# brucefan1983/GPUMD

Measured on AMD Instinct MI355X. Metric: atom-steps/sec, NEP PbTe NVE (nep4 2 Te Pb, examples/nep_train/nep.txt), higher is better.
Workload: dtype f32

## Files before the change

### gpumd_amd/csrc/capi_impl.h

```cpp
#pragma once
#include "../../include/nepmi.h"
#include "engine_impl.h"

#include <exception>
#include <string>

struct nepmi_api;
#if defined(NEPMI_CAPI_DISPATCH)
extern "C" const nepmi_api nepmi_self_api;
#define NEPMI_SELF_API (&nepmi_self_api)
#else
#define NEPMI_SELF_API nullptr
#endif

struct nepmi_model {
  const nepmi_api* api;
  nepmi::NepModel m;
};

struct nepmi_engine {
  const nepmi_api* api;
  nepmi::EngineT<NepmiBackend>* e;
};

// ... 903 lines not shown
int nepmi_engine_set_option(nepmi_engine* e, const char* name, double value)
{
  if (!e || !name)
    return fail(NEPMI_ERR_ARG, "null engine or option name");
  const std::string n(name);
  const int iv = (int)value;
  auto& eng = *e->e;
  if (n == "generic")
    return guarded([&] { eng.set_force_generic(iv != 0); });
  if (n == "tiles")
    eng.set_tile_mode(iv < 0 ? -1 : iv > 2 ? 2 : iv);
  else if (n == "win_lanes")
    eng.set_win_lanes(iv);
  else if (n == "win_max_atoms")
    eng.set_win_max_atoms(iv);
  else if (n == "scatter_guard")
    eng.set_scatter_guard_delayed(value, eng.take_guard_delay());
  else if (n == "scatter_guard_hard")
    eng.set_scatter_guard(-1.0, value);
  else if (n == "scatter_guard_delay")
    eng.set_guard_delay(iv);
  else if (n == "radial_mask")
    eng.set_radial_mask(iv != 0);
  else if (n == "radial_sync")
    eng.set_radial_sync(iv != 0);
  else if (n == "angular_fused")
    eng.set_angular_fused(iv != 0);
  else if (n == "angular_pair_trip")
    eng.set_angular_pair_trip(iv != 0);
  else if (n == "angular_flat_tables")
    eng.set_angular_flat_tables(iv != 0);
  else if (n == "lean_list_walks")
    eng.set_lean_list_walks(iv != 0);
  else if (n == "fold_seam")
    eng.set_fold_seam(iv != 0);
  else if (n == "brick_force") {
    if (iv != 0 && !eng.has_brick_force())
      return fail(NEPMI_ERR_ARG, "option 'brick_force': the per-brick force kernel is not part of this build (make BRICK=1)");
    eng.set_brick_force(iv != 0);
  }
  else if (n == "win_static")
    eng.set_win2(iv != 0);
  else if (n == "keep_lists_on_box_change")
    eng.set_keep_lists(iv != 0);
  else if (n == "stepwise_loops")
    eng.set_stepwise_loops(iv != 0);
  else if (n == "mfma")
    eng.set_use_mfma(iv);
  else if (n == "angular_recompute")
    eng.set_angular_recompute(iv);
  else
    return fail(NEPMI_ERR_ARG, "unknown engine option '" + n + "'");
  return NEPMI_OK;
}

}
```

### gpumd_amd/csrc/engine_impl.h

```cpp
#pragma once
#include "nep_bodies.h"
#include "nep_md.h"
#include "nep_corr.h"
#include "nep_rdf.h"
#include "nep_adf.h"
#include "nep_model.h"
#include "nep_window.h"
#include "nep_highl.h"
#include "tersoff_bodies.h"

#include <cmath>
#include <cstdio>
#include <cstring>
#include <string>
#include <random>
#include <vector>

#ifndef NEPMI_TERSOFF_SEAM
#define NEPMI_TERSOFF_SEAM 1
#endif
#ifndef NEPMI_WIN2_DEFAULT
#define NEPMI_WIN2_DEFAULT 1
#endif

// ... 1216 lines not shown
    b_.posq = dalloc<PosQ>(N);
    b_.x0s = dalloc<double>(3 * N);
    b_.nn_skin = dalloc<int>(N);
    b_.nl_skin = dalloc<int>((size_t)b_.MN_skin * N);
    b_.code_skin = dalloc<unsigned short>((size_t)b_.MN_skin * N);
    b_.nn_ang = dalloc<int>(N);
    b_.nl_ang = dalloc<int>((size_t)b_.MN_ang * N);
    b_.code_ang = dalloc<unsigned short>((size_t)b_.MN_ang * N);
    b_.rev_ang = dalloc<unsigned short>((size_t)b_.MN_ang * N);
    b_.nn_rad = dalloc<int>(N);
    b_.nn_angstep = dalloc<int>(N);
    b_.nn_angtrue = dalloc<int>(N);
    if (m.kind == 0) {
      b_.rstash = dalloc<F4>((size_t)(b_.MN_ang + b_.MN_skin) * N);
      b_.acomp = dalloc<F4>((size_t)b_.MN_arows * N);
      b_.amap = dalloc<unsigned short>((size_t)b_.MN_ang * N);
      b_.f12 = dalloc<F4>((size_t)b_.MN_arows * N);
      b_.q = dalloc<float>((size_t)m.dim * N);
      b_.fp = dalloc<float>((size_t)m.dim * N);
      b_.sbuf = dalloc<float>((size_t)(m.n_max_angular + 1) * kNumHarm * N);
      b_.shi = m.L_max > 4 ? dalloc<float>((size_t)(m.n_max_angular + 1) * kHighSums * N) : nullptr;
      b_.KRP = ((m.basis_size_radial + 1) + 3) / 4 * 4;
      b_.atab = dalloc<float>((size_t)N * m.num_types * b_.KRP);
      const AnnMfmaShape as = ann_mfma_shape(m.num_types, m.dim, m.num_neurons, b_.KRP);
      b_.ann_img = as.ok ? dalloc<float>(as.img_floats * m.num_types) : nullptr;
      be_.ann_prepare(md_, b_);
      b_.pe_i = dalloc<float>(N);
      b_.MN_rad = m.MN_radial;
      b_.ccode = dalloc<unsigned short>((size_t)b_.MN_rad * N);
      b_.nn_t0 = dalloc<int>(N);
      b_.prec = dalloc<WinRec>(N);
      b_.aidx = dalloc<unsigned short>((size_t)b_.MN_acomp * N);
      b_.amask = dalloc<unsigned>(4 * (size_t)N);
      b_.MN_wchunks = (b_.MN_ang + 3) / 4 + 2 * ((b_.MN_skin + 3) / 4) + 4;
      b_.wcode = dalloc<unsigned short>((size_t)b_.MN_wchunks * 4 * N);
      b_.wseg = dalloc<int>(N);
      b_.FPR = (m.n_max_radial + 1 + 3) / 4 * 4;
      b_.fpr = (m.num_types > 4 || !served_by_type_pure_shape(m)) ? dalloc<float>((size_t)N * b_.FPR) : nullptr;
      b_.MN_cw = (b_.MN_rad + 3) / 4 + 1;
      b_.cword = dalloc<unsigned short>((size_t)2 * b_.MN_cw * 4 * N);
      b_.aslot = B::kHasScatter ? dalloc<unsigned short>((size_t)b_.MN_arows * N) : nullptr;
      b_.compact_all = b_.aslot ? 1 : 0;
      b_.MAW = (4 * ((b_.MN_ang + 3) / 4) + 31) / 32 + 1;
      b_.MBW = (8 * ((b_.MN_skin + 3) / 4) + 31) / 32 + 1;
      b_.rmaskA = B::kHasScatter ? dalloc<unsigned>((size_t)b_.MAW * N) : nullptr;
      b_.rmaskB = B::kHasScatter ? dalloc<unsigned>((size_t)b_.MBW * N) : nullptr;
      b_.tmaskA = B::kHasScatter ? dalloc<unsigned>((size_t)b_.MAW * N) : nullptr;
      b_.MA2 = 2 * ((b_.MN_ang + 3) / 4) + 2;
      const bool two = B::kHasScatter && m.num_types == 2;
      b_.acode2 = two ? dalloc<unsigned short>((size_t)b_.MA2 * N * 4) : nullptr;
      b_.aorig2 = two ? dalloc<unsigned>((size_t)b_.MA2 * N) : nullptr;
      b_.aseg2 = two ? dalloc<int>(N) : nullptr;
      b_.use_rmask = 0;
      b_.use_csync = 0;
    } else {
      tb_.rec = dalloc<D4>((size_t)b_.MN_ang * N);
      tb_.bb = dalloc<double>((size_t)b_.MN_ang * N);
      tb_.bp = dalloc<double>((size_t)b_.MN_ang * N);
      tb_.f12 = dalloc<D4>((size_t)b_.MN_ang * N);
      tb_.pe_d = dalloc<double>(N);
      tb_.mask = dalloc<unsigned long long>(N);
      for (int k = 0; k < 3; ++k) {
        const TersoffSet& s = m.ters[k];
        tp_.p[k] = TersoffSetD{s.a, s.b, s.lambda, s.mu, s.beta, s.n, s.c, s.d, s.h, s.r1, s.r2, s.c2, s.d2,
                               s.one_plus_c2overd2, s.pi_factor, s.minus_half_over_n};
      }
      tp_.rc_sq = (float)(m.rc_radial_max * m.rc_radial_max);
// ... 260 lines not shown
      build_in_windows = flags[kFlagMaxCell] <= 127 && flags[kFlagMaxWindow] <= win_max_atoms() && !flags[kFlagOutlier];
      for (int d = 0; d < 3; ++d)
        if (box_.pbc[d] && nb[d] < 8)
          build_in_windows = false;
      if (build_in_windows) {
        WinLayout lay = win_;
        lay.wmax = (flags[kFlagMaxWindow] + 63) / 64 * 64;
        lay.compact = 0;
        be_.launch_win(kSlotMisc, num_bricks_, BuildListsWinBody{WinStage{box_, b_, lay}});
      }
    }
    if (!build_in_windows)
      be_.template launch<128>(kSlotMisc, N_, BuildListsBody{box_, b_});
    rev_valid_ = false;
    if (model_.kind == 1 || b_.level)
      ensure_reverse_slots();
    be_.end_region(kRegionRebuild);
    be_.d2h(flags, b_.flags, sizeof(flags));
    check_overflow(flags);
    num_boundary_bricks_ = flags[kFlagNumBoundary];
    max_ang_rebuild_ = flags[kFlagMaxAng];
    tile_ok_ = use_tiles_ && model_.kind == 0 && flags[kFlagMaxCell] <= 127 && flags[kFlagMaxWindow] <= win_max_atoms() &&
               !flags[kFlagOutlier];
    for (int d = 0; d < 3; ++d)
      if (box_.pbc[d] && nb[d] < 8)
        tile_ok_ = false;
    if (std::getenv("NEPMI_DEBUG_REBUILD"))
      std::fprintf(stderr, "nepmi rebuild: cells %d %d %d max_cell %d max_window %d (cap %d) max_brick %d outlier %d tiles %d -> tile_ok %d\n", nb[0], nb[1], nb[2],
                   flags[kFlagMaxCell], flags[kFlagMaxWindow], win_max_atoms(), flags[kFlagMaxBrick], flags[kFlagOutlier], (int)use_tiles_, (int)tile_ok_);
    win_.wmax = (flags[kFlagMaxWindow] + 63) / 64 * 64;
    win2_ok_ = tile_ok_ && use_win2_ && b_.wtab != nullptr && win_.wmax < 65535;
    if (win2_ok_) {
      b_.wsent = win_.wmax;
      be_.template launch<128>(kSlotMisc, N_, PackCodesBody{b_, shape_ts() == 2 ? 2 : 1});
      be_.d2h(flags, b_.flags, sizeof(flags));
      check_overflow(flags);
    }
    if (win2_ok_ && b_.aslot) {
      const size_t need = (size_t)num_bricks_ * (size_t)win_.wmax * kHaloRowWords;
      if (need > halo_cap_) {
        dfree(halo_);
        halo_ = nullptr;
        halo_ = dalloc<int>(need + need / 8);
        halo_cap_ = need + need / 8;
      }
      if (!fmap_)
        fmap_ = dalloc<unsigned>((size_t)fold_rows_ * cap_);
      fold_ok_ = num_bricks_ < ((int64_t)1 << 19) && win_.wmax < (1 << 13);
      if (fold_ok_) {
        int most = be_.build_fold_map(N_, box_, b_, win_.wmax, fold_rows_, fmap_);
        if (most > fold_rows_) {
          fold_rows_ = most;
          dfree(fmap_);
          fmap_ = nullptr;
          fmap_ = dalloc<unsigned>((size_t)fold_rows_ * cap_);
          most = be_.build_fold_map(N_, box_, b_, win_.wmax, fold_rows_, fmap_);
        }
      }
    }
    if (reverse_ghosts_ && b_.level) {
      be_.memset(b_.atab, 0, sizeof(float) * (size_t)cap_ * model_.num_types * b_.KRP);
      be_.memset(b_.f12, 0, sizeof(F4) * (size_t)b_.MN_arows * cap_);
      if (b_.fpr)
        be_.memset(b_.fpr, 0, sizeof(float) * (size_t)cap_ * b_.FPR);
    }
    have_list_ = true;
    ++num_rebuild;
// ... 299 lines not shown
    if (!m.temperature_model || m.kind != 0 || temperature == temperature_)
      return;
    temperature_ = temperature;
    const float qT = (float)temperature * m.q_scaler_temp;
    b0_eff_.resize(m.b0.size());
    for (size_t k = 0; k < m.b0.size(); ++k)
      b0_eff_[k] = m.b0[k] - m.w0_temp[k] * qT;
    be_.h2d(const_cast<float*>(md_.b0), b0_eff_.data(), sizeof(float) * b0_eff_.size());
    be_.ann_prepare(md_, b_);
    fused_img_stale_ = fused_img_flat_stale_ = true;
  }
  double temperature() const { return temperature_; }
  bool temperature_model() const { return model_.temperature_model; }
  int recompute_s() const
  {
    return recompute_mode_ < 0 ? (model_.MN_angular <= 16 ? 1 : 0) : (recompute_mode_ ? 1 : 0);
  }
  void adopt_from(const EngineT& o)
  {
    use_tiles_ = o.use_tiles_;
    tile_mode_ = o.tile_mode_;
    recompute_mode_ = o.recompute_mode_;
    win_lanes_ = o.win_lanes_;
    win_max_atoms_ = o.win_max_atoms_;
    use_win2_ = o.use_win2_;
    external_skin_ = o.external_skin_;
    force_form_ = o.force_form_;
    use_rmask_ = o.use_rmask_;
    use_csync_ = o.use_csync_;
    ang_fused_ = o.ang_fused_;
    ang_pair_trip_ = o.ang_pair_trip_;
    ang_flat_tables_ = o.ang_flat_tables_;
    lean_walks_ = o.lean_walks_;
    fold_seam_ = o.fold_seam_;
    brick_force_ = o.brick_force_;
    loop_ctx_ = o.loop_ctx_;
    scatter_disabled_ = o.scatter_disabled_;
    b_.scatter_limit = o.b_.scatter_limit;
    b_.fold_guard = o.b_.fold_guard;
    b_.scatter_hard = o.b_.scatter_hard;
    b_.fold_hard = o.b_.fold_hard;
    hard_factor_ = o.hard_factor_;
    hard_asked_ = o.hard_asked_;
    guard_delay_ = o.guard_delay_;
    guard_delayed_ = o.guard_delayed_;
    if (reverse_ghosts_ != o.reverse_ghosts_)
      set_reverse_ghosts(o.reverse_ghosts_);
    unwrapped_ = o.unwrapped_;
    nhc_fresh_ = o.nhc_fresh_;
    bdp_rng_ = o.bdp_rng_;
    bdp_iset_ = o.bdp_iset_;
    bdp_gset_ = o.bdp_gset_;
    lan_seed_ = o.lan_seed_;
    num_compute = o.num_compute;
    num_rebuild = o.num_rebuild;
    num_discarded = o.num_discarded;
    num_range_handovers = o.num_range_handovers;
    be_.adopt_options(o.be_);
    if (ann_mode_ != o.ann_mode_)
      set_use_mfma(o.ann_mode_);
    if (force_generic_ != o.force_generic_)
      set_force_generic(o.force_generic_);
    if (o.temperature_ != temperature_)
      set_temperature(o.temperature_);
    have_list_ = false;
  }
// ... 45 lines not shown
      be_.template launch<64>(kSlotMisc, N_, RadialDescBody<S>{box_, md_, b_, 1});
      records_valid_ = true;
      return;
    }
    const int lanes = win_lanes();
    const bool win2 = win2_ok_ && lanes == 1;
    last_rows_form_ = false;
    last_fpj_form_ = false;
    if (phase != kPhaseRadialOnly) {
      WinLayout layq = win_;
      layq.compact = 1;
      const WinStage wsq{box_, b_, layq};
      b_.use_rmask = (NEPMI_RMASK && use_rmask_ && S::TS > 0 && win2 && b_.rmaskB && loop_ctx_ && max_ang_rebuild_ <= 96 &&
                      (S::TS == 1 || b_.acode2) && scatter_wanted<S>(wsq))
                       ? 1
                       : 0;
      last_mask_form_ = b_.use_rmask != 0;
      b_.use_csync = (NEPMI_CSYNC && use_csync_ && !b_.use_rmask && win2 && b_.cword && loop_ctx_ && b_.MN_cw < 256 &&
                      scatter_wanted<S>(wsq))
                       ? 1
                       : 0;
      last_sync_form_ = b_.use_csync != 0;
    } else {
      b_.use_rmask = 0;
      b_.use_csync = 0;
    }
    WinLayout lay2 = win_;
    lay2.compact = 1;
    const WinStage ws2{box_, b_, lay2};
    if (!(win2 && b_.use_csync && S::fixed))
      ensure_reverse_slots();
    B& rbe = radial_side_ ? *radial_side_ : be_;
    auto radial = [&](int64_t nb, int first) {
      if (win2 && b_.use_csync && lean_radial<S>())
        rbe.launch_win2(kSlotRadial, nb, RadialWin2Body<S, 1, 1>{ws2, md_, first, frozen});
      else if (win2 && b_.use_csync)
        rbe.launch_win2(kSlotRadial, nb, RadialWin2Body<S, 1>{ws2, md_, first, frozen});
      else if (win2 && lean_radial<S>())
        rbe.launch_win2(kSlotRadial, nb, RadialWin2Body<S, 0, 1>{ws2, md_, first, frozen});
      else if (win2)
        rbe.launch_win2(kSlotRadial, nb, RadialWin2Body<S>{ws2, md_, first, frozen});
      else if (lanes == 4)
        rbe.launch_win_split(kSlotRadial, nb, RadialWinSplitBody<S, 4>{ws, md_, first, frozen});
      else if (lanes == 2)
        rbe.launch_win_split(kSlotRadial, nb, RadialWinSplitBody<S, 2>{ws, md_, first, frozen});
      else
        rbe.launch_win(kSlotRadial, nb, RadialWinBody<S>{ws, md_, first, frozen});
    };
    if (phase == kPhaseRadialOnly) {
      b_.use_rmask = 0;
      b_.use_csync = 0;
      if (tile_ok_)
        radial(num_bricks_, -1);
      ccode_valid_ = true;
      return;
    }
    if (phase == kPhaseInterior) {
      radial(num_bricks_ - num_boundary_bricks_, 0);
      return;
    }
    if (phase == kPhaseBoundaryRadial) {
      radial(num_boundary_bricks_, (int)(num_bricks_ - num_boundary_bricks_));
      return;
    }
    records_valid_ = !tile_ok_;
    be_.begin_region(kRegionForce);
// ... 146 lines not shown
      fold_deferred_ = true;
    } else {
      be_.template launch_force_scatter<S>(kSlotForce, num_bricks_, -1, N_, ws2, md_, halo_, fmap_, fold_rows_, step_outputs_,
                                           list_mode(), 0, 2, frozen);
    }
    if (!step_outputs_)
      outputs_stale_ = true;
    last_scatter_form_ = true;
    return true;
  }
  template <class S>
  void assembly_rest_shape(const int* frozen)
  {
    WinLayout lay2 = win_;
    lay2.compact = 1;
    const WinStage ws2{box_, b_, lay2};
    be_.template launch_force_scatter<S>(kSlotForce, num_bricks_ - num_boundary_bricks_, 0, N_, ws2, md_, halo_, fmap_, fold_rows_,
                                         pending_outputs_, list_mode(), 2, 2, frozen);
  }

public:
  void set_force_form(int mode) { force_form_ = mode < 0 ? -1 : (mode > 1 ? 1 : mode); }
  void set_assembly_part(int part) { assembly_part_ = part; }
  bool assembly_pending() const { return assembly_pending_; }
  void force_assembly_rest(const int* frozen)
  {
    if (!assembly_pending_)
      return;
    assembly_pending_ = false;
    be_.frozen = frozen;
    NEPMI_SHAPE_DISPATCH(assembly_rest_shape, 1, (frozen))
    be_.frozen = nullptr;
  }
  void set_radial_mask(bool on) { use_rmask_ = on; }
  void set_radial_sync(bool on) { use_csync_ = on; }
  void set_scatter_guard(double limit, double hard_factor = 4.0)
  {
    if (limit < 0.0)
      limit = b_.scatter_limit;
    if (hard_factor >= 0.0)
      hard_asked_ = hard_factor;
    if (!(limit > 0.0) || limit > 64.0)
      limit = 64.0;
    hard_factor = hard_asked_;
    if (!(hard_factor >= 1.0) || hard_factor * limit > 256.0)
      hard_factor = 256.0 / limit < 4.0 ? 256.0 / limit : 4.0;
    b_.scatter_limit = (float)limit;
    b_.fold_guard = (int)(2.0 * limit * 4194304.0);
    hard_factor_ = hard_factor;
    if (b_.scatter_hard > 0.0f)
      set_flagged_steps_stand(true);
  }
  double scatter_guard() const { return b_.scatter_limit; }
  void set_scatter_guard_delayed(double limit, int n)
  {
    if (n <= 0) {
      set_scatter_guard(limit, -1.0);
      return;
    }
    guard_delayed_ = limit;
    guard_delay_ = n;
  }
  void set_guard_delay(int n) { guard_delay_next_ = n > 0 ? n : 0; }
  int take_guard_delay()
  {
    const int n = guard_delay_next_;
    guard_delay_next_ = 0;
    return n;
  }
  void set_flagged_steps_stand(bool on)
  {
    b_.scatter_hard = on ? (float)(hard_factor_ * b_.scatter_limit) : 0.0f;
    b_.fold_hard = on ? (int)((hard_factor_ > 2.0 ? hard_factor_ : 2.0) * b_.scatter_limit * 4194304.0) : 0;
  }
  bool scatter_enabled() const { return !scatter_disabled_; }
  void clear_range_hard()
  {
    int ov = 0;
    be_.d2h(&ov, b_.flags + kFlagOverflow, sizeof(int));
    if (ov & kOverflowRangeHard) {
      ov &= ~kOverflowRangeHard;
      be_.h2d(b_.flags + kFlagOverflow, &ov, sizeof(int));
    }
  }
  void disable_scatter()
  {
    if (!scatter_disabled_)
      ++num_range_handovers;
    scatter_disabled_ = true;
    be_.memset(b_.flags + kFlagRange, 0, sizeof(int));
  }
  bool last_scatter_form() const { return last_scatter_form_; }
  void set_angular_fused(bool on) { ang_fused_ = on; }
  void set_angular_pair_trip(bool on) { ang_pair_trip_ = on; }
  bool ang_pair_trip_active() const { return ang_pair_trip_ && (model_.n_max_angular + 2) / 2 <= 4; }
  void set_angular_flat_tables(bool on) { ang_flat_tables_ = on; }
  void set_lean_list_walks(bool on) { lean_walks_ = on; }
  template <class S>
  bool lean_radial() const
  {
    return lean_walks_ && S::TS > 0;
  }
  bool lean_scatter() const { return lean_walks_ && shape_ts() > 0; }
  void set_fold_seam(bool on) { fold_seam_ = on; }
  void set_brick_force(bool on) { brick_force_ = on; }
  static constexpr bool has_brick_force() { return B::kHasBrickForce; }
  void set_loop_context(bool on) { loop_ctx_ = on; }
  void set_step_outputs(bool on) { step_outputs_ = on; }
  bool loop_context() const { return loop_ctx_; }
  void exact_virials()
  {
    if (!virial_local_ || model_.kind != 0 || last_small_)
      return;
    be_.frozen = nullptr;
    NEPMI_SHAPE_DISPATCH(exact_virials_shape, 1, ())
  }
  bool virial_local() const { return virial_local_; }

private:
  template <class S>
  void compact_lists_shape()
  {
    const bool padded_rows = b_.use_csync != 0;
    force_kernels_shape<S>(kPhaseRadialOnly, nullptr);
    if (padded_rows)
      angular_kernels<S>();
  }
  template <class S>
  void exact_virials_shape()
  {
// ... 72 lines not shown
          char eb[128];
          std::snprintf(eb, sizeof eb, "<-zero_padded_model(%d,%d,%d,%d,%d)", model_.file_n_max_radial, model_.file_basis_size_radial,
                        model_.file_n_max_angular, model_.file_basis_size_angular, model_.file_num_L);
          s += eb;
        }
      } else {
        s += std::string("shape=") + shapes[shape_ >= 0 && shape_ <= 5 ? shape_ : 0];
      }
    }
    if (last_small_)
      return s + " path=small_box(all image pairs)";
    const int lanes = win_lanes();
    const bool win2 = win2_ok_ && lanes == 1;
    s += tile_ok_ ? (win2 ? " window=lds_static" : " window=lds_scanned") : " window=none(gather kernels)";
    s += " lanes_per_atom=" + std::to_string(tile_ok_ ? lanes : 1);
    if (last_brick_)
      s += " force=one_kernel_per_brick(descriptor+ann+partial_forces+lds_scatter_of_own_halves,lane_pairs)";
    else if (last_ang_fused_ && last_ang_window_)
      s += " angular=descriptor+ann+partial_forces_in_one_kernel(lane_pairs,sums_in_registers,type_sorted,window_of_4_types)";
    else if (last_ang_fused_)
      s += std::string(" angular=descriptor+ann+partial_forces_in_one_kernel(lane_pairs,sums_in_registers") +
           (ang_pair_trip_active() ? ",two_record_trips" : "") + (last_ang_flat_ ? ",flat_tables)" : ")");
    else if (fuse_ann_active())
      s += " ann=fused_with_angular_descriptor(packed_fp32,no_mfma)";
    else if (ann_mode_ != 0 && b_.ann_img && (model_.num_types <= 4 || b_.skip_atab))
      s += model_.num_types > 4 ? " ann=mfma_f32_32x32x2(one_type_per_workgroup)" : " ann=mfma_f32_32x32x2";
    else
      s += " ann=per_atom";
    if (!last_ang_fused_) {
      s += (shape_ != 0 && model_.n_max_angular + 1 >= 7) ? " angular_force=lane_pairs" : " angular_force=one_lane";
      s += recompute_s() ? " angular_sums=recomputed" : " angular_sums=stored";
    }
    s += (tile_ok_ && win2 && shape_ts() > 0 && lean_walks_) ? " list_walks=lean" : " list_walks=classic";
    s += (last_scatter_form_ && last_mask_form_)   ? " radial_list=inside_bits_over_the_verlet_words"
         : (last_scatter_form_ && last_sync_form_) ? " radial_list=wave_synchronous_words"
                                                   : " radial_list=compacted";
    s += last_scatter_form_ ? (last_fold_seam_ ? " force_assembly=lds_scatter_of_own_halves(fixed_point)+fold_in_integrator_pass"
                                               : " force_assembly=lds_scatter_of_own_halves(fixed_point)+fold") :
         last_rows_form_ ? " force_assembly=table_rows_in_lds"
                         : (last_fpj_form_ ? " force_assembly=neighbour_half_from_fp_rows" : " force_assembly=table_rows_gathered");
    if (num_seam_vetoes_ > 0)
      s += " seam_vetoes=" + std::to_string(num_seam_vetoes_);
    if (tile_ok_)
      s += " bricks=" + std::to_string(num_bricks_) + " window_slots=" + std::to_string(win_.wmax);
    return s;
  }
  void force_kernels(int phase, const int* frozen = nullptr)
  {
    be_.frozen = frozen;
    force_kernels_dispatch(phase, frozen);
    be_.frozen = nullptr;
    step_outputs_ = true;
    assembly_part_ = 0;
  }
  void force_kernels_on(B& side, int phase, const int* frozen)
  {
    if (phase != kPhaseBoundaryRadial || !tile_ok_)
      throw EngineError{-4, "force_kernels_on: the boundary bricks' radial pass of the window kernels only"};
    radial_side_ = &side;
    side.frozen = frozen;
    force_kernels_dispatch(phase, frozen);
    side.frozen = nullptr;
    radial_side_ = nullptr;
  }

private:
// ... 4 lines not shown
      if (N_ < 200000)
        be_.template launch_lds_parts<kTersoffBlock, kTersoffLanes>(kSlotRadial, N_, TersoffPartialBody{box_, tp_, b_, tb_, kTersoffLanes});
      else
        be_.template launch_lds<kTersoffBlock>(kSlotRadial, N_, TersoffPartialBody{box_, tp_, b_, tb_});
      if (tersoff_defer_)
        tersoff_deferred_ = true;
      else
        be_.template launch<64>(kSlotForce, N_, TersoffAssembleBody{b_, tb_});
      be_.end_region(kRegionForce);
      return;
    }
    NEPMI_SHAPE_DISPATCH(force_kernels_shape, 1, (phase, frozen))
  }

  NepModel model_;
  B be_;
  int64_t cap_;
  int64_t N_;
  ModelD md_{};
  Bufs b_;
  BoxD box_;
  WinLayout win_{0, 0};
  bool win2_ok_ = false, use_win2_ = NEPMI_WIN2_DEFAULT != 0;
  bool use_rows_ = true;
  bool last_rows_form_ = false, last_fpj_form_ = false, last_scatter_form_ = false;
  int force_form_ = -1;
  bool loop_ctx_ = false;
  bool virial_local_ = false;
  double hard_factor_ = 4.0;
  bool ang_fused_ = true;
  bool ang_pair_trip_ = !(std::getenv("NEPMI_ANGULAR_PAIR_TRIP") && std::atoi(std::getenv("NEPMI_ANGULAR_PAIR_TRIP")) == 0);
  bool ang_flat_tables_ = !(std::getenv("NEPMI_ANGULAR_FLAT_TABLES") && std::atoi(std::getenv("NEPMI_ANGULAR_FLAT_TABLES")) == 0);
  bool lean_walks_ = !(std::getenv("NEPMI_LEAN_LIST_WALKS") && std::atoi(std::getenv("NEPMI_LEAN_LIST_WALKS")) == 0);
  float* fused_img_flat_ = nullptr;
  size_t fused_img_flat_floats_ = 0;
  bool fused_img_flat_stale_ = true;
  bool last_ang_flat_ = false;
  bool brick_force_ = false;
  bool last_brick_ = false;
  bool brick_pending_ = false;
  float* fused_img_ = nullptr;
  size_t fused_img_floats_ = 0;
  bool fused_img_stale_ = true;
  bool last_ang_fused_ = false;
  bool use_rmask_ = false;
  bool last_mask_form_ = false;
  bool last_ang_window_ = false;
  bool last_sync_form_ = false;
  int guard_delay_ = 0;
  int guard_delay_next_ = 0;
  bool fold_seam_ = !(std::getenv("NEPMI_FOLD_SEAM") && std::atoi(std::getenv("NEPMI_FOLD_SEAM")) == 0);
  bool fold_defer_ = false;
  bool fold_deferred_ = false;
  static constexpr int kSeamBackoffSteps = 256;
  int seam_backoff_ = 0;
  int64_t num_seam_vetoes_ = 0;
  bool last_fold_seam_ = false;
  bool tersoff_defer_ = false;
  bool tersoff_deferred_ = false;
  int64_t calm_steps_ = 0;
  int* brick_live_buf_ = nullptr;
  double* thermo_rows_ = nullptr;
  int64_t thermo_rows_cap_ = 0;
  bool rev_valid_ = false;
  const int* dmap_dev_ = nullptr;
  double hard_asked_ = 4.0;
// ... 77 lines not shown
```

### gpumd_amd/csrc/nep_bodies.h

```cpp
#pragma once
#include <type_traits>

#include "nep_dev.h"

namespace nepmi {

struct alignas(16) F4 {
  float x, y, z;
  int w;
};

struct alignas(16) U4 {
  unsigned x, y, z, w;
};

struct alignas(16) WinRec {
  int x, y, z;
  int w;
};

struct WinGeom {
  double inv_unit;
  double cell_frac[3];
  int cv[9];
// ... 793 lines not shown
  }
};

struct MarkGhostCellsBody {
  Bufs b;
  NEPMI_HD void operator()(int64_t k) const
  {
    if (b.lvl[k] < 2)
      b.cell_ghost[b.kcell[k]] = 1;
    if (b.lvl[k] >= 1 && b.brick_live)
      b.brick_live[b.kcell[k] >> 6] = 1;
  }
};
struct BrickOrderBody {
  Bufs b;
  int64_t nbricks;
  NEPMI_HD void operator()(int64_t brick) const
  {
    const int before = b.brick_flag[brick];
    const int nbound = b.brick_flag[nbricks];
    const bool boundary = b.brick_flag[brick + 1] != before;
    if (boundary)
      b.brick_order[(nbricks - nbound) + before] = (int)brick;
    else
      b.brick_order[brick - before] = (int)brick;
    if (brick == 0)
      b.flags[kFlagNumBoundary] = nbound;
  }
};

struct PackCodesBody {
  Bufs b;
  int parts;
  NEPMI_HD void operator()(int64_t k) const
  {
    const int64_t N = b.N;
    const int64_t brick = b.kcell[k] >> 6;
    const int* tab = b.wtab + brick * 1024;
    unsigned short* out = b.wcode + k * 4;
    const int64_t row = N * 4;
    int word = 0, fill = 0;
    unsigned short cur[4];
    auto put = [&](unsigned short slot) {
      cur[fill++] = slot;
      if (fill == 4) {
        if (word < b.MN_wchunks)
          for (int u = 0; u < 4; ++u)
            out[(int64_t)word * row + u] = cur[u];
        ++word;
        fill = 0;
      }
    };
    auto flush = [&]() {
      while (fill != 0)
        put((unsigned short)b.wsent);
    };
    auto slot_of = [&](unsigned code) { return (unsigned short)((tab[(code >> 7) * 2 + 1] & 0xFFFF) + (code & 127u)); };
    const int na = b.nn_ang[k], nb = b.nn_skin[k];
    for (int s = 0; s < na; ++s)
      put(slot_of(b.code_ang[(int64_t)s * N + k]));
    flush();
    const int wa = word;
    if (b.tmaskA && parts == 2) {
      for (int w = 0; w < b.MAW; ++w) {
        unsigned bits = 0u;
        for (int s = 32 * w; s < na && s < 32 * w + 32; ++s)
// ... 11 lines not shown
          if (row2 < b.MA2) {
            for (int u = 0; u < 4; ++u)
              b.acode2[((int64_t)row2 * N + k) * 4 + u] = sl[u];
            b.aorig2[(int64_t)row2 * N + k] = ix;
          }
          ++row2;
          f2 = 0;
          ix = 0u;
        };
        for (int s2 = 0; s2 < na; ++s2) {
          if ((b.posq[b.nl_ang[(int64_t)s2 * N + k]].type != 0) != (t != 0))
            continue;
          sl[f2] = slot_of(b.code_ang[(int64_t)s2 * N + k]);
          ix |= (unsigned)(s2 < 255 ? s2 : 255) << (8 * f2);
          if (++f2 == 4)
            emit();
        }
        if (f2 != 0) {
          for (; f2 < 4; ++f2) {
            sl[f2] = (unsigned short)b.wsent;
            ix |= 255u << (8 * f2);
          }
          emit();
        }
        if (t == 0)
          wa0 = row2;
      }
      if (row2 > b.MA2 || na > 255)
        NEPMI_ATOMIC_OR(&b.flags[kFlagOverflow], 1);
      b.aseg2[k] = wa0 | ((row2 - wa0) << 8);
    }
    int wb = 0;
    if (parts == 2) {
      int s0 = 0, s1 = 0;
      unsigned long long m0 = 0ull, m1 = 0ull, m2 = 0ull, m3 = 0ull;
      const bool masked = nb <= 256;
      if (masked)
        for (int s = 0; s < nb; ++s) {
          const unsigned long long bit = (b.posq[b.nl_skin[(int64_t)s * N + k]].type != 0 ? 1ull : 0ull) << (s & 63);
          const int w = s >> 6;
          m0 |= w == 0 ? bit : 0ull;
          m1 |= w == 1 ? bit : 0ull;
          m2 |= w == 2 ? bit : 0ull;
          m3 |= w == 3 ? bit : 0ull;
        }
      auto other = [&](int s) -> bool {
        const int w = s >> 6;
        const unsigned long long m = w == 0 ? m0 : (w == 1 ? m1 : (w == 2 ? m2 : m3));
        return ((m >> (s & 63)) & 1ull) != 0ull;
      };
      auto next_of = [&](int& s, int want) -> int {
        if (masked) {
          while (s < nb && other(s) != (want != 0))
            ++s;
        } else {
          while (s < nb && (b.posq[b.nl_skin[(int64_t)s * N + k]].type != 0) != (want != 0))
            ++s;
        }
        return s < nb ? s++ : -1;
      };
      for (;;) {
        int e0[4], e1[4];
        for (int u = 0; u < 4; ++u)
          e0[u] = next_of(s0, 0);
        for (int u = 0; u < 4; ++u)
          e1[u] = next_of(s1, 1);
        if (e0[0] < 0 && e1[0] < 0)
          break;
        for (int u = 0; u < 4; ++u)
          put(e0[u] >= 0 ? slot_of(b.code_skin[(int64_t)e0[u] * N + k]) : (unsigned short)b.wsent);
        for (int u = 0; u < 4; ++u)
          put(e1[u] >= 0 ? slot_of(b.code_skin[(int64_t)e1[u] * N + k]) : (unsigned short)b.wsent);
        ++wb;
      }
    } else {
      for (int s = 0; s < nb; ++s)
        put(slot_of(b.code_skin[(int64_t)s * N + k]));
      flush();
      wb = word - wa;
    }
    if (word > b.MN_wchunks || wa > 255 || wb > 255)
      NEPMI_ATOMIC_OR(&b.flags[kFlagOverflow], 1);
    b.wseg[k] = wa | (wb << 8);
  }
};

struct CheckGatherBody {
  BoxD box;
  Bufs b;
  const double* pos;
  int which;
  NEPMI_HD void operator()(int64_t k) const
  {
#pragma clang fp contract(off)
    const int64_t N = b.N;
    if (which != 0 && (b.lvl[k] >= 2) != (which == 1))
      return;
    const int64_t i = b.perm[k];
    const double x = pos[i], y = pos[N + i], z = pos[2 * N + i];
    float dx = (float)(x - b.x0s[k]);
    float dy = (float)(y - b.x0s[N + k]);
    float dz = (float)(z - b.x0s[2 * N + k]);
    int n0, n1, n2;
    mic_f_img(box, dx, dy, dz, n0, n1, n2);
    const float d2 = (dx * dx + dy * dy) + dz * dz;
// ... 1583 lines not shown
```

### gpumd_amd/csrc/nep_window.h

```cpp
#pragma once
#include "nep_bodies.h"

namespace nepmi {

constexpr int kWinThreads = 256;
#ifndef NEPMI_BIGWIN_RADIAL
#define NEPMI_BIGWIN_RADIAL 1024
#endif
#ifndef NEPMI_BIGWIN_SCATTER
#define NEPMI_BIGWIN_SCATTER 768
#endif
constexpr int kWinThreadsBig = NEPMI_BIGWIN_RADIAL;
constexpr int kWinThreadsBigScatter = NEPMI_BIGWIN_SCATTER;
constexpr size_t kBigWindowLds = 80 * 1024;
#ifndef NEPMI_MIDWIN
#define NEPMI_MIDWIN 1
#endif
constexpr int kWinThreadsMid = 512;
constexpr size_t kMidWindowLds = 54 * 1024;
constexpr int kWinCells = 512;
constexpr int kWinMaxAtoms = 6656;

#if defined(__HIP_DEVICE_COMPILE__)
#define NEPMI_LDS(T) __attribute__((address_space(3))) T
// ... 723 lines not shown
    f3 = funnel16(slot, f3);
    ++p;
  }
  NEPMI_HD unsigned pop_one(unsigned sent)
  {
    if (p <= 0)
      return sent;
    const int s = 8 - p;
    const unsigned r01 = (s & 2) ? f1 : f0, r23 = (s & 2) ? f3 : f2;
    const unsigned r = (s & 4) ? r23 : r01;
    --p;
    return (s & 1) ? (r >> 16) : (r & 0xFFFFu);
  }
  NEPMI_HD unsigned long long pop_word(unsigned long long sent64)
  {
    const int s = 8 - p;
    const unsigned long long lo01 = ((unsigned long long)f1 << 32) | f0, hi23 = ((unsigned long long)f3 << 32) | f2;
    const unsigned long long lo = (s & 4) ? hi23 : lo01, hi = (s & 4) ? 0ull : hi23;
    const int sh = 16 * (s & 3);
    unsigned long long w = sh ? ((lo >> sh) | (hi << (64 - sh))) : lo;
    if (p < 4) {
      const unsigned long long keep = (1ull << (16 * p)) - 1ull;
      w = (w & keep) | (sent64 & ~keep);
      p = 0;
    } else {
      p -= 4;
    }
    return w;
  }
};

constexpr int kListModeLean = 4;

template <class S, int SYNC = 0, int LEAN = 0>
struct RadialWin2Body {
  WinStage st;
  ModelD m;
  int first;
  const int* frozen;
  static constexpr int kMinWavesPerEu = NEPMI_RW2_WAVES;
  static constexpr bool kBigWindows = S::TS > 0;
  static constexpr bool kMidWindows = NEPMI_MIDWIN != 0 && S::TS == 0 && S::fixed && SYNC != 0;

  NEPMI_HD int ctab_floats() const { return S::TS > 0 ? 0 : m.T * m.T * ctab_block(m.NR, m.KR, false); }
  NEPMI_HD int ctab_offset() const { return (st.lay.bytes() + 15) / 16 * 16; }
  NEPMI_HD bool ctab_on() const { return NEPMI_RW_CTAB && S::TS == 0 && ctab_offset() + 4 * ctab_floats() <= 80 * 1024; }
  NEPMI_HD int lds_bytes() const { return ctab_on() ? ctab_offset() + 4 * ctab_floats() : st.lay.bytes(); }
  NEPMI_HD int64_t map_brick(int64_t w) const { return first < 0 ? w : (int64_t)st.b.brick_order[first + w]; }
  NEPMI_HD bool skip() const { return frozen && *frozen != 0; }
  template <class LC>
  NEPMI_HD void stage(int64_t brick, LC lds, int tid, int nth) const
  {
    if (st.b.brick_live && !st.b.brick_live[brick])
      return;
    st.stage_direct(brick, lds, tid, nth);
    if (ctab_on())
      ctab_stage_padded(m, lds + ctab_offset(), tid, nth, false);
  }
  NEPMI_HD void brick_range(int64_t brick, int64_t& a0, int64_t& a1) const { st.brick_range(brick, a0, a1); }

  template <class LC>
  NEPMI_HD void compute(int64_t brick, int64_t k, LC lds) const
  {
    const Bufs& b = st.b;
    const int64_t N = b.N;
    if (b.lvl[k] < 1) {
      b.nn_rad[k] = 0;
      b.nn_angstep[k] = 0;
// ... 39 lines not shown
      const WinRec r = wrec[slot];
      c.slot = slot;
      c.rw = r.w;
      c.fx = (float)(r.x - ox);
      c.fy = (float)(r.y - oy);
      c.fz = (float)(r.z - oz);
      c.d2 = dot3f(c.fx, c.fx, c.fy, c.fy, c.fz, c.fz) * unit2;
      const int t2 = (int)((unsigned)r.w >> kIdxBits);
      const float rc = m.uniform_rc ? m.rc_r_max : (rc1 + m.rc_r[t2]) * 0.5f;
      const float er = c.d2 - rc * rc;
      c.inside = er < 0.0f;
      float near = fabsf(er);
      c.ang = false;
      if (list_a) {
        const float rca = m.uniform_rc ? m.rc_a_max : (rca1 + m.rc_a[t2]) * 0.5f;
        const float ea = c.d2 - rca * rca;
        c.ang = ea < 0.0f;
        near = fminf(near, fabsf(ea));
      }
      nearband = nearband || near < band;
      return c;
    };
    auto retake = [&](Cand& c, bool list_a) __attribute__((always_inline)) {
      const int t2 = (int)((unsigned)c.rw >> kIdxBits);
      const float rc = m.uniform_rc ? m.rc_r_max : (rc1 + m.rc_r[t2]) * 0.5f;
      const float rca = m.uniform_rc ? m.rc_a_max : (rca1 + m.rc_a[t2]) * 0.5f;
      const float er = c.d2 - rc * rc, ea = c.d2 - rca * rca;
      const float near = list_a ? fminf(fabsf(er), fabsf(ea)) : fabsf(er);
      if (near < band && c.slot != b.wsent) {
        float ex, ey, ez;
        const float d2e = pair_geometry(st.box, p1, b.posq[(unsigned)c.rw & (unsigned)kIdxMask], ex, ey, ez);
        c.inside = d2e < rc * rc;
        c.ang = list_a && d2e < rca * rca;
      }
    };
    U2w* __restrict__ cword = reinterpret_cast<U2w*>(b.cword) + k;
    unsigned long long accf = 0ull, accb = 0ull;
    unsigned mcur = 0u;
    auto accumulate1 = [&](const Cand& c) __attribute__((always_inline)) {
      if (!c.inside)
        return;
      const int t2 = (int)((unsigned)c.rw >> kIdxBits);
      const float rc = m.uniform_rc ? m.rc_r_max : (rc1 + m.rc_r[t2]) * 0.5f;
      float d, dinv;
      dist_and_inv(c.d2, d, dinv);
      const float rcinv = fast_rcp(rc);
      const float dc = d < rc ? d : rc;
      float fc;
      cutoff_fc(rcinv, dc, fc);
      float fn[S::KRM + 1];
      if (S::fixed)
        basis_fn<S::KRM>(rcinv, dc, fc, fn);
      else
        basis_fn_rt(KR, rcinv, dc, fc, fn);
      if (ctab) {
        float g[S::NRM + 1];
        ctab_contract<S, false>(ctab_lds + (t1 * m.T + t2) * ctab_block(NR, KR, false), NR, KR, fn, g);
#pragma unroll
        for (int n = 0; n <= S::NRM; ++n) {
          if (!S::fixed && n > NR)
            break;
          q[n] += g[n];
        }
      } else {
        const float* cc = m.c_rad + (t1 * m.T + t2) * (NR + 1) * (KR + 1);
        for (int n = 0; n <= NR; ++n) {
// ... 199 lines not shown
      dist_and_inv(c0.d2, d0, i0);
      dist_and_inv(c1.d2, d1, i1);
      const f2 dc = LEAN ? mk2(clamp_to_cutoff(d0, rc0), clamp_to_cutoff(d1, rc1v)) : mk2(d0 < rc0 ? d0 : rc0, d1 < rc1v ? d1 : rc1v);
      const f2 rcinv = mk2(ri0, ri1);
      f2 fc;
      cutoff_fc_v(rcinv, dc, fc);
      fc = fc * mk2(c0.inside ? 1.0f : 0.0f, c1.inside ? 1.0f : 0.0f);
      basis_fn_v<S::KRM>(rcinv, dc, fc, fn);
    };

    f2 SS[S::KRM + 1];
#pragma unroll
    for (int kk = 0; kk <= S::KRM; ++kk)
      SS[kk] = bc2(0.0f);

    auto load_word = [&](int w, int wend) __attribute__((always_inline)) -> U2w {
      U2w v = {0u, 0u};
      if (wend > 0)
        v = words[(int64_t)(w < wend ? w : wend - 1) * N];
      return v;
    };

    {
      U2w w1 = load_word(0, wa), w2 = load_word(1, wa);
      for (int w = 0; w < wa; ++w) {
        const U2w cur = w1;
        w1 = w2;
        w2 = load_word(w + 2, wa);
#pragma unroll
        for (int hh = 0; hh < 2; ++hh) {
          const unsigned pr = hh == 0 ? cur.lo : cur.hi;
          bool nearband = false;
          Cand c[2];
          c[0] = judge((int)(pr & 0xFFFFu), true, nearband);
          c[1] = judge((int)(pr >> 16), true, nearband);
          if (nearband) {
            retake(c[0], true);
            retake(c[1], true);
          }
          if (ASYNC) {
            while (NEPMI_WAVE_ANY(qa.p > 6))
              ang_emit();
          }
#pragma unroll
          for (int u = 0; u < 2; ++u) {
            const int idx = 4 * w + 2 * hh + u;
            const bool live = idx < na;
            unsigned short cs = kNoSlot;
            if (ASYNC) {
              if (c[u].ang) {
                qa.push((unsigned)c[u].slot);
                ++ca;
              }
            } else if (c[u].ang) {
              if (ca < b.MN_acomp) {
                F4 e;
                e.x = c[u].fx * unit;
                e.y = c[u].fy * unit;
                e.z = c[u].fz * unit;
                e.w = c[u].rw;
                if (NEPMI_RW2_ABL != 3) {
                  acomp[(int64_t)ca * N] = e;
                  aidx[(int64_t)ca * N] = b.rev_ang[(int64_t)idx * N + k];
                  if (b.aslot)
                    b.aslot[(int64_t)ca * N + k] = (unsigned short)c[u].slot;
                }
                cs = (unsigned short)ca;
                const unsigned bit = 1u << (idx & 31);
                const int aw = idx >> 5;
                am[0] |= aw == 0 ? bit : 0u;
                am[1] |= aw == 1 ? bit : 0u;
                am[2] |= aw == 2 ? bit : 0u;
                am[3] |= aw == 3 ? bit : 0u;
              }
              ++ca;
            }
            if (!ASYNC && !b.use_amask && live)
              amap[(int64_t)idx * N] = cs;
            if (S::TS == 2 && ((unsigned)c[u].rw >> kIdxBits) == 1u)
              push_back(c[u], 4 * (w & 7) + 2 * hh + u);
            else
              push_front(c[u], 4 * (w & 7) + 2 * hh + u);
          }
          if (S::TS > 0 && !ZIP) {
            f2 fn[S::KRM + 1];
            basis2(c[0], c[1], fn);
#pragma unroll
            for (int kk = 0; kk <= S::KRM; ++kk)
              SS[kk] = SS[kk] + fn[kk];
          } else if (ZIP && LEAN) {
            f2 fn[S::KRM + 1];
            basis2(c[0], c[1], fn);
            const bool one0 = ((unsigned)c[0].rw >> kIdxBits) == 1u, one1 = ((unsigned)c[1].rw >> kIdxBits) == 1u;
            const f2 wt0 = mk2(one0 ? 0.0f : 1.0f, one0 ? 1.0f : 0.0f), wt1 = mk2(one1 ? 0.0f : 1.0f, one1 ? 1.0f : 0.0f);
#pragma unroll
            for (int kk = 0; kk <= S::KRM; ++kk) {
              SS[kk] = vfma(wt0, bc2(fn[kk].x), SS[kk]);
              SS[kk] = vfma(wt1, bc2(fn[kk].y), SS[kk]);
            }
          } else if (ZIP) {
#pragma unroll
            for (int u = 0; u < 2; ++u) {
              f2 fn[S::KRM + 1];
              basis2(c[u], c[u], fn);
              const bool one = ((unsigned)c[u].rw >> kIdxBits) == 1u;
              const f2 wt = mk2(one ? 0.0f : 1.0f, one ? 1.0f : 0.0f);
#pragma unroll
              for (int kk = 0; kk <= S::KRM; ++kk)
                SS[kk] = vfma(wt, fn[kk], SS[kk]);
            }
          } else if (wide) {
            accumulate_wide(c, 2);
          } else {
            accumulate1(c[0]);
            accumulate1(c[1]);
          }
        }
        if (!SYNC && b.use_rmask && ((w & 7) == 7 || w == wa - 1)) {
          if ((w >> 3) < b.MAW)
            b.rmaskA[(int64_t)(w >> 3) * N + k] = mcur;
          mcur = 0u;
        }
        sync_check();
      }
    }
    if (ASYNC) {
      while (NEPMI_WAVE_ANY(qa.p > 0))
        ang_emit();
    } else if (b.use_amask) {
      U4 mv;
      mv.x = am[0];
      mv.y = am[1];
      mv.z = am[2];
      mv.w = am[3];
      reinterpret_cast<U4*>(b.amask)[k] = mv;
    }

    if (ZIP) {
      const int rows = 2 * wb;
      U2w a1 = load_word(wa, wa + rows), b1 = load_word(wa + 1, wa + rows);
      U2w a2 = load_word(wa + 2, wa + rows), b2 = load_word(wa + 3, wa + rows);
      for (int p = 0; p < wb; ++p) {
        const U2w ca0 = a1, cb0 = b1;
        a1 = a2;
        b1 = b2;
        a2 = load_word(wa + 2 * p + 4, wa + rows);
        b2 = load_word(wa + 2 * p + 5, wa + rows);
        constexpr int HN = NEPMI_RW2_HALF ? 2 : 4;
#pragma unroll
        for (int hh = 0; hh < 4 / HN; ++hh) {
// ... 977 lines not shown
```

### gpumd_amd/dist.py

```python
import ctypes as C

import numpy as np

from . import _capi

ENSEMBLES = {"nve": 0, "nvt_ber": 1, "nvt_nhc": 2, "nvt_bdp": 3, "nvt_lan": 4, "nvt_bao": 5}


def choose_grid(world):
    best = (world, 1, 1)
    for a in range(1, world + 1):
        if world % a:
            continue
        for b in range(1, world // a + 1):
            if (world // a) % b:
                continue
            c = world // a // b
            g = tuple(sorted((a, b, c), reverse=True))
            if max(g) - min(g) < max(best) - min(best):
                best = g
    return best


class Transport:
# ... 90 lines not shown
    def lan_seed(self, seed):
        self._ck(self.lib.nepmi_dist_lan_seed(self.handle, int(seed)))

    def set_overlap(self, on=True):
        self._ck(self.lib.nepmi_dist_set_overlap(self.handle, 1 if on else 0))

    def num_overlapped_reverse(self):
        return int(self.lib.nepmi_dist_num_overlapped_reverse(self.handle))

    def info(self):
        assert self.lib.nepmi_dist_info_bytes() == C.sizeof(_capi.NepmiDistInfo)
        out = _capi.NepmiDistInfo()
        self._ck(self.lib.nepmi_dist_get_info(self.handle, C.byref(out)))
        return out

    def gather_owned(self, ids, pos, vel, force, pe=None, virial=None):
        self._ck(self.lib.nepmi_dist_gather_owned(self.handle, self._ptr(ids), self._ptr(pos), self._ptr(vel),
                                                  self._ptr(force), self._ptr(pe), self._ptr(virial)))

    def gather_global(self, root, pos=None, vel=None, force=None, pe=None, virial=None):
        self._ck(self.lib.nepmi_dist_gather_global(self.handle, int(root), self._ptr(pos), self._ptr(vel), self._ptr(force),
                                                   self._ptr(pe), self._ptr(virial)))

    def engine_stats(self, with_lists=False):
        e = self.lib.nepmi_dist_engine(self.handle)
        st = _capi.NepmiStats()
        self._ck(self.lib.nepmi_engine_stats(e, 1 if with_lists else 0, C.byref(st)))
        return st

    def engine_set_timing(self, mode):
        self._ck(self.lib.nepmi_engine_set_timing(self.lib.nepmi_dist_engine(self.handle), int(mode)))

    def engine_describe(self):
        buf = C.create_string_buffer(512)
        n = self.lib.nepmi_engine_describe(self.lib.nepmi_dist_engine(self.handle), buf, 512)
        return buf.value.decode() if n >= 0 else ""
```

### gpumd_amd/nep.py

```python
import ctypes as C
import weakref

import numpy as np

from . import _capi


def _h9(box):
    h = np.ascontiguousarray(np.asarray(box, dtype=np.float64).reshape(9))
    return h, h.ctypes.data_as(_capi.c_dp)


def _pbc3(pbc):
    p = np.ascontiguousarray(np.asarray(pbc, dtype=np.int32).reshape(3))
    return p, p.ctypes.data_as(_capi.c_ip)


class Model:

    def __init__(self, path, lib=None):
        from . import load_library
        self.lib = lib if lib is not None else load_library()
        self.path = path
        self.handle = self.lib.nepmi_model_load(path.encode())
# ... 304 lines not shown
        self.set_option("win_lanes", int(lanes))

    def set_force_form(self, mode=-1):
        self._ck(self.lib.nepmi_engine_set_force_form(self.handle, int(mode)))

    def set_radial_mask(self, on=True):
        self.set_option("radial_mask", 1 if on else 0)

    def set_radial_sync(self, on=True):
        self.set_option("radial_sync", 1 if on else 0)

    def set_scatter_guard(self, ev_per_angstrom=64.0, hard_factor=0.0):
        self.set_option("scatter_guard", float(ev_per_angstrom))
        self.set_option("scatter_guard_hard", float(hard_factor))

    def set_virial_mode(self, mode=0):
        self._ck(self.lib.nepmi_engine_set_virial_mode(self.handle, int(mode)))

    def set_brick_force(self, on=True):
        self.set_option("brick_force", 1 if on else 0)

    def set_angular_fused(self, on=True):
        self.set_option("angular_fused", 1 if on else 0)

    def set_angular_pair_trip(self, on=True):
        self.set_option("angular_pair_trip", 1 if on else 0)

    def set_angular_flat_tables(self, on=True):
        self.set_option("angular_flat_tables", 1 if on else 0)

    def set_lean_list_walks(self, on=True):
        self.set_option("lean_list_walks", 1 if on else 0)

    def set_fold_seam(self, on=True):
        self.set_option("fold_seam", 1 if on else 0)

    def describe(self):
        import ctypes as C
        buf = C.create_string_buffer(512)
        n = self.lib.nepmi_engine_describe(self.handle, buf, 512)
        if n < 0:
            self._ck(n)
        return buf.value.decode()

    def set_stepwise_loops(self, on=True):
        self.set_option("stepwise_loops", int(bool(on)))

    def set_win_static(self, on=True):
        self.set_option("win_static", int(bool(on)))

    def set_mfma(self, on=True):
        self.set_option("mfma", int(on))

    def set_temperature(self, temperature):
        self._ck(self.lib.nepmi_engine_set_temperature(self.handle, float(temperature)))

    def set_angular_recompute(self, mode=-1):
        self.set_option("angular_recompute", int(mode))

    def set_generic(self, on=True):
        self.set_option("generic", 1 if on else 0)


def dos_from_mvac(lib, sums, group_size, dt_ps, omega_max, num_dos_points=None):
    sums = np.ascontiguousarray(sums, dtype=np.float64)
    ng, _, nc = sums.shape
    npts = nc if num_dos_points is None else int(num_dos_points)
    size = np.ascontiguousarray(group_size, dtype=np.int64)
    if sums.shape[1] != 3 or size.shape != (ng,):
        raise ValueError("sums: [G, 3, Nc], group_size: [G]")
    mvac, dos = np.zeros((ng, 3, nc)), np.zeros((ng, 3, max(npts, 0)))
    _capi.check(lib, lib.nepmi_dos_from_mvac(sums.ctypes.data_as(_capi.c_dp), ng, nc, size.ctypes.data_as(C.POINTER(_capi.c_i64)),
                                             float(dt_ps), float(omega_max), npts, mvac.ctypes.data_as(_capi.c_dp),
# ... 206 lines not shown
```

Before: 995.3 million.

## Walk list A for angular membership only in two-type radial window pass

For two-type models, the radial window kernel gets an AONLY variant. It judges list A entries only against the angular cutoff and skips radial accumulation and pushes for them. The pack-codes kernel then folds list A entries into the radial stream alongside the skin list, so radial work runs over one type-sorted stream. This aims to remove duplicated radial checks and the split handling of list A. In exchange the word-chunk buffer grows, and correctness depends on the combined packing covering all radial neighbours. It is on by default and references a macro NEPMI_RW2_ABL that is not shown.

```diff
diff --git a/gpumd_amd/csrc/capi_impl.h b/gpumd_amd/csrc/capi_impl.h
--- a/gpumd_amd/csrc/capi_impl.h
+++ b/gpumd_amd/csrc/capi_impl.h
@@ -959,6 +959,8 @@
     eng.set_angular_flat_tables(iv != 0);
   else if (n == "lean_list_walks")
     eng.set_lean_list_walks(iv != 0);
+  else if (n == "angular_only_list_a")
+    eng.set_angular_only_list_a(iv != 0);
   else if (n == "fold_seam")
     eng.set_fold_seam(iv != 0);
   else if (n == "brick_force") {
diff --git a/gpumd_amd/csrc/engine_impl.h b/gpumd_amd/csrc/engine_impl.h
--- a/gpumd_amd/csrc/engine_impl.h
+++ b/gpumd_amd/csrc/engine_impl.h
@@ -1272,7 +1272,7 @@
       b_.prec = dalloc<WinRec>(N);
       b_.aidx = dalloc<unsigned short>((size_t)b_.MN_acomp * N);
       b_.amask = dalloc<unsigned>(4 * (size_t)N);
-      b_.MN_wchunks = (b_.MN_ang + 3) / 4 + 2 * ((b_.MN_skin + 3) / 4) + 4;
+      b_.MN_wchunks = (b_.MN_ang + 3) / 4 + 2 * (((m.num_types == 2 ? b_.MN_ang : 0) + b_.MN_skin + 3) / 4) + 4;
       b_.wcode = dalloc<unsigned short>((size_t)b_.MN_wchunks * 4 * N);
       b_.wseg = dalloc<int>(N);
       b_.FPR = (m.n_max_radial + 1 + 3) / 4 * 4;
@@ -1599,7 +1599,8 @@
     win2_ok_ = tile_ok_ && use_win2_ && b_.wtab != nullptr && win_.wmax < 65535;
     if (win2_ok_) {
       b_.wsent = win_.wmax;
-      be_.template launch<128>(kSlotMisc, N_, PackCodesBody{b_, shape_ts() == 2 ? 2 : 1});
+      aonly_built_ = aonly_list_a_active();
+      be_.template launch<128>(kSlotMisc, N_, PackCodesBody{b_, shape_ts() == 2 ? 2 : 1, (aonly_built_ && NEPMI_RW2_ABL != 4) ? 1 : 0});
       be_.d2h(flags, b_.flags, sizeof(flags));
       check_overflow(flags);
     }
@@ -1965,6 +1966,7 @@
     ang_pair_trip_ = o.ang_pair_trip_;
     ang_flat_tables_ = o.ang_flat_tables_;
     lean_walks_ = o.lean_walks_;
+    aonly_list_a_ = o.aonly_list_a_;
     fold_seam_ = o.fold_seam_;
     brick_force_ = o.brick_force_;
     loop_ctx_ = o.loop_ctx_;
@@ -2076,6 +2078,19 @@
       ensure_reverse_slots();
     B& rbe = radial_side_ ? *radial_side_ : be_;
     auto radial = [&](int64_t nb, int first) {
+      if constexpr (S::TS == 2) {
+        if (win2 && aonly_built_ && !b_.use_rmask) {
+          if (b_.use_csync && lean_radial<S>())
+            rbe.launch_win2(kSlotRadial, nb, RadialWin2Body<S, 1, 1, 1>{ws2, md_, first, frozen});
+          else if (b_.use_csync)
+            rbe.launch_win2(kSlotRadial, nb, RadialWin2Body<S, 1, 0, 1>{ws2, md_, first, frozen});
+          else if (lean_radial<S>())
+            rbe.launch_win2(kSlotRadial, nb, RadialWin2Body<S, 0, 1, 1>{ws2, md_, first, frozen});
+          else
+            rbe.launch_win2(kSlotRadial, nb, RadialWin2Body<S, 0, 0, 1>{ws2, md_, first, frozen});
+          return;
+        }
+      }
       if (win2 && b_.use_csync && lean_radial<S>())
         rbe.launch_win2(kSlotRadial, nb, RadialWin2Body<S, 1, 1>{ws2, md_, first, frozen});
       else if (win2 && b_.use_csync)
@@ -2288,7 +2303,12 @@
     NEPMI_SHAPE_DISPATCH(assembly_rest_shape, 1, (frozen))
     be_.frozen = nullptr;
   }
-  void set_radial_mask(bool on) { use_rmask_ = on; }
+  void set_radial_mask(bool on)
+  {
+    if (on != use_rmask_ && aonly_list_a_)
+      have_list_ = false;
+    use_rmask_ = on;
+  }
   void set_radial_sync(bool on) { use_csync_ = on; }
   void set_scatter_guard(double limit, double hard_factor = 4.0)
   {
@@ -2352,6 +2372,13 @@
   bool ang_pair_trip_active() const { return ang_pair_trip_ && (model_.n_max_angular + 2) / 2 <= 4; }
   void set_angular_flat_tables(bool on) { ang_flat_tables_ = on; }
   void set_lean_list_walks(bool on) { lean_walks_ = on; }
+  void set_angular_only_list_a(bool on)
+  {
+    if (on != aonly_list_a_)
+      have_list_ = false;
+    aonly_list_a_ = on;
+  }
+  bool aonly_list_a_active() const { return aonly_list_a_ && shape_ts() == 2 && !use_rmask_; }
   template <class S>
   bool lean_radial() const
   {
@@ -2490,6 +2517,7 @@
       s += recompute_s() ? " angular_sums=recomputed" : " angular_sums=stored";
     }
     s += (tile_ok_ && win2 && shape_ts() > 0 && lean_walks_) ? " list_walks=lean" : " list_walks=classic";
+    s += (tile_ok_ && win2 && aonly_built_) ? " list_a=angular_only" : " list_a=classic";
     s += (last_scatter_form_ && last_mask_form_)   ? " radial_list=inside_bits_over_the_verlet_words"
          : (last_scatter_form_ && last_sync_form_) ? " radial_list=wave_synchronous_words"
                                                    : " radial_list=compacted";
@@ -2560,6 +2588,8 @@
   bool ang_pair_trip_ = !(std::getenv("NEPMI_ANGULAR_PAIR_TRIP") && std::atoi(std::getenv("NEPMI_ANGULAR_PAIR_TRIP")) == 0);
   bool ang_flat_tables_ = !(std::getenv("NEPMI_ANGULAR_FLAT_TABLES") && std::atoi(std::getenv("NEPMI_ANGULAR_FLAT_TABLES")) == 0);
   bool lean_walks_ = !(std::getenv("NEPMI_LEAN_LIST_WALKS") && std::atoi(std::getenv("NEPMI_LEAN_LIST_WALKS")) == 0);
+  bool aonly_list_a_ = !(std::getenv("NEPMI_ANGULAR_ONLY_LIST_A") && std::atoi(std::getenv("NEPMI_ANGULAR_ONLY_LIST_A")) == 0);
+  bool aonly_built_ = false;
   float* fused_img_flat_ = nullptr;
   size_t fused_img_flat_floats_ = 0;
   bool fused_img_flat_stale_ = true;
diff --git a/gpumd_amd/csrc/nep_bodies.h b/gpumd_amd/csrc/nep_bodies.h
--- a/gpumd_amd/csrc/nep_bodies.h
+++ b/gpumd_amd/csrc/nep_bodies.h
@@ -849,6 +849,7 @@
 struct PackCodesBody {
   Bufs b;
   int parts;
+  int aonly;
   NEPMI_HD void operator()(int64_t k) const
   {
     const int64_t N = b.N;
@@ -926,12 +927,19 @@
     }
     int wb = 0;
     if (parts == 2) {
+      const int n0 = aonly ? na : 0, nv = n0 + nb;
+      auto type_of = [&](int s) -> bool {
+        return b.posq[s < n0 ? b.nl_ang[(int64_t)s * N + k] : b.nl_skin[(int64_t)(s - n0) * N + k]].type != 0;
+      };
+      auto code_of = [&](int s) -> unsigned {
+        return s < n0 ? b.code_ang[(int64_t)s * N + k] : b.code_skin[(int64_t)(s - n0) * N + k];
+      };
       int s0 = 0, s1 = 0;
       unsigned long long m0 = 0ull, m1 = 0ull, m2 = 0ull, m3 = 0ull;
-      const bool masked = nb <= 256;
+      const bool masked = nv <= 256;
       if (masked)
-        for (int s = 0; s < nb; ++s) {
-          const unsigned long long bit = (b.posq[b.nl_skin[(int64_t)s * N + k]].type != 0 ? 1ull : 0ull) << (s & 63);
+        for (int s = 0; s < nv; ++s) {
+          const unsigned long long bit = (type_of(s) ? 1ull : 0ull) << (s & 63);
           const int w = s >> 6;
           m0 |= w == 0 ? bit : 0ull;
           m1 |= w == 1 ? bit : 0ull;
@@ -945,13 +953,13 @@
       };
       auto next_of = [&](int& s, int want) -> int {
         if (masked) {
-          while (s < nb && other(s) != (want != 0))
+          while (s < nv && other(s) != (want != 0))
             ++s;
         } else {
-          while (s < nb && (b.posq[b.nl_skin[(int64_t)s * N + k]].type != 0) != (want != 0))
+          while (s < nv && type_of(s) != (want != 0))
             ++s;
         }
-        return s < nb ? s++ : -1;
+        return s < nv ? s++ : -1;
       };
       for (;;) {
         int e0[4], e1[4];
@@ -962,9 +970,9 @@
         if (e0[0] < 0 && e1[0] < 0)
           break;
         for (int u = 0; u < 4; ++u)
-          put(e0[u] >= 0 ? slot_of(b.code_skin[(int64_t)e0[u] * N + k]) : (unsigned short)b.wsent);
+          put(e0[u] >= 0 ? slot_of(code_of(e0[u])) : (unsigned short)b.wsent);
         for (int u = 0; u < 4; ++u)
-          put(e1[u] >= 0 ? slot_of(b.code_skin[(int64_t)e1[u] * N + k]) : (unsigned short)b.wsent);
+          put(e1[u] >= 0 ? slot_of(code_of(e1[u])) : (unsigned short)b.wsent);
         ++wb;
       }
     } else {
diff --git a/gpumd_amd/csrc/nep_window.h b/gpumd_amd/csrc/nep_window.h
--- a/gpumd_amd/csrc/nep_window.h
+++ b/gpumd_amd/csrc/nep_window.h
@@ -779,8 +779,9 @@
 
 constexpr int kListModeLean = 4;
 
-template <class S, int SYNC = 0, int LEAN = 0>
+template <class S, int SYNC = 0, int LEAN = 0, int AONLY = 0>
 struct RadialWin2Body {
+  static_assert(AONLY == 0 || S::TS == 2, "AONLY: two-type shapes only");
   WinStage st;
   ModelD m;
   int first;
@@ -886,6 +887,30 @@
         const float d2e = pair_geometry(st.box, p1, b.posq[(unsigned)c.rw & (unsigned)kIdxMask], ex, ey, ez);
         c.inside = d2e < rc * rc;
         c.ang = list_a && d2e < rca * rca;
+      }
+    };
+    auto judge_ang = [&](int slot, bool& nearband) __attribute__((always_inline)) -> Cand {
+      Cand c;
+      const WinRec r = wrec[slot];
+      c.slot = slot;
+      c.rw = r.w;
+      c.fx = (float)(r.x - ox);
+      c.fy = (float)(r.y - oy);
+      c.fz = (float)(r.z - oz);
+      c.d2 = dot3f(c.fx, c.fx, c.fy, c.fy, c.fz, c.fz) * unit2;
+      const float rca = m.uniform_rc ? m.rc_a_max : (rca1 + m.rc_a[(unsigned)r.w >> kIdxBits]) * 0.5f;
+      const float ea = c.d2 - rca * rca;
+      c.inside = false;
+      c.ang = ea < 0.0f;
+      nearband = nearband || fabsf(ea) < band;
+      return c;
+    };
+    auto retake_ang = [&](Cand& c) __attribute__((always_inline)) {
+      const float rca = m.uniform_rc ? m.rc_a_max : (rca1 + m.rc_a[(unsigned)c.rw >> kIdxBits]) * 0.5f;
+      if (fabsf(c.d2 - rca * rca) < band && c.slot != b.wsent) {
+        float ex, ey, ez;
+        const float d2e = pair_geometry(st.box, p1, b.posq[(unsigned)c.rw & (unsigned)kIdxMask], ex, ey, ez);
+        c.ang = d2e < rca * rca;
       }
     };
     U2w* __restrict__ cword = reinterpret_cast<U2w*>(b.cword) + k;
@@ -1151,11 +1176,20 @@
           const unsigned pr = hh == 0 ? cur.lo : cur.hi;
           bool nearband = false;
           Cand c[2];
-          c[0] = judge((int)(pr & 0xFFFFu), true, nearband);
-          c[1] = judge((int)(pr >> 16), true, nearband);
-          if (nearband) {
-            retake(c[0], true);
-            retake(c[1], true);
+          if (AONLY) {
+            c[0] = judge_ang((int)(pr & 0xFFFFu), nearband);
+            c[1] = judge_ang((int)(pr >> 16), nearband);
+            if (nearband) {
+              retake_ang(c[0]);
+              retake_ang(c[1]);
+            }
+          } else {
+            c[0] = judge((int)(pr & 0xFFFFu), true, nearband);
+            c[1] = judge((int)(pr >> 16), true, nearband);
+            if (nearband) {
+              retake(c[0], true);
+              retake(c[1], true);
+            }
           }
           if (ASYNC) {
             while (NEPMI_WAVE_ANY(qa.p > 6))
@@ -1196,12 +1230,15 @@
             }
             if (!ASYNC && !b.use_amask && live)
               amap[(int64_t)idx * N] = cs;
+            if (AONLY)
+              continue;
             if (S::TS == 2 && ((unsigned)c[u].rw >> kIdxBits) == 1u)
               push_back(c[u], 4 * (w & 7) + 2 * hh + u);
             else
               push_front(c[u], 4 * (w & 7) + 2 * hh + u);
           }
-          if (S::TS > 0 && !ZIP) {
+          if (AONLY) {
+          } else if (S::TS > 0 && !ZIP) {
             f2 fn[S::KRM + 1];
             basis2(c[0], c[1], fn);
 #pragma unroll
@@ -1235,6 +1272,8 @@
             accumulate1(c[1]);
           }
         }
+        if (AONLY)
+          continue;
         if (!SYNC && b.use_rmask && ((w & 7) == 7 || w == wa - 1)) {
           if ((w >> 3) < b.MAW)
             b.rmaskA[(int64_t)(w >> 3) * N + k] = mcur;
diff --git a/gpumd_amd/dist.py b/gpumd_amd/dist.py
--- a/gpumd_amd/dist.py
+++ b/gpumd_amd/dist.py
@@ -146,6 +146,6 @@
         self._ck(self.lib.nepmi_engine_set_timing(self.lib.nepmi_dist_engine(self.handle), int(mode)))
 
     def engine_describe(self):
-        buf = C.create_string_buffer(512)
-        n = self.lib.nepmi_engine_describe(self.lib.nepmi_dist_engine(self.handle), buf, 512)
+        buf = C.create_string_buffer(1024)
+        n = self.lib.nepmi_engine_describe(self.lib.nepmi_dist_engine(self.handle), buf, 1024)
         return buf.value.decode() if n >= 0 else ""
diff --git a/gpumd_amd/nep.py b/gpumd_amd/nep.py
--- a/gpumd_amd/nep.py
+++ b/gpumd_amd/nep.py
@@ -360,13 +360,16 @@
     def set_lean_list_walks(self, on=True):
         self.set_option("lean_list_walks", 1 if on else 0)
 
+    def set_angular_only_list_a(self, on=True):
+        self.set_option("angular_only_list_a", 1 if on else 0)
+
     def set_fold_seam(self, on=True):
         self.set_option("fold_seam", 1 if on else 0)
 
     def describe(self):
         import ctypes as C
-        buf = C.create_string_buffer(512)
-        n = self.lib.nepmi_engine_describe(self.handle, buf, 512)
+        buf = C.create_string_buffer(1024)
+        n = self.lib.nepmi_engine_describe(self.handle, buf, 1024)
         if n < 0:
             self._ck(n)
         return buf.value.decode()
```

Measured after the change: 1.016 billion, median of 6. 2.1% higher.
